# AY-Liu/Image-Editing-Framework

Hardware: AMD Instinct MI355X
Metric: denoising steps/sec (SD1.5 512x512 P2P edit step, UNet batch 4) (higher is better)
Workload: dtype f16x3; 1 GPU; sd15 UNet (859.5M params) P2P AttentionRefine edit step, 2 prompts x CFG = batch 4, 64x64 latents (512x512 px), 50-step DDIM, guidance 7.5, cross 0.8 / self 0.4, per-step null-text unconditional embeddings (P2P_NTI, edit_real.py); one independent edit per GPU; precision mode f16x3: fp32 storage; every contraction on split operands: hi + lo fp16 halves of each fp32 element, Ah Bh + Al Bh + Ah Bl =

## Files before the change

### image-editing-framework_amd/control.py

```python
from typing import Optional

import torch

from . import hip

XL = 96


def _step_hook(c):
    fn = getattr(c, "between_steps", None) or getattr(c, "after_step", None)
    if fn is not None:
        fn()


def advance_controller(c):
    c.cur_att_layer += 1
    uncond = c.num_att_layers if getattr(c, "LOW_RESOURCE", False) else 0
    if c.cur_att_layer == c.num_att_layers + uncond:
        c.cur_att_layer = 0
        c.cur_step += 1
        _step_hook(c)


class StepCounter:
# ... 21 lines not shown
        self.cond_only = bool(cond_only)
        self.batch = num_prompts if cond_only else 2 * num_prompts
        self.num_steps = num_steps
        self.self_window = self_window
        self.self_max_tokens = self_max_tokens
        self.captured = False
        self.muted = False
        dev = self.device
        self.step = torch.zeros(1, dtype=torch.int32, device=dev)
        B, Bp = self.batch, num_prompts
        if kind == "p2p":
            slots = Bp - 1
            assert mt.shape == (slots, XL, XL) and coef_table.shape == (num_steps + 1, slots, 2, XL)
            self.mt = mt.to(device=dev, dtype=torch.float16).contiguous()
            self.mt32 = mt.to(device=dev, dtype=torch.float32).contiguous()
            self.coef_table = coef_table.to(device=dev, dtype=torch.float32).contiguous()
            self.coef_cur = torch.zeros(slots, 2, XL, dtype=torch.float32, device=dev)
            ct = coef_table.detach().float()
            self.coef_bound = float((ct[:, :, 0].abs() + ct[:, :, 1].abs()).max()) if ct.numel() else 1.0
            off = 0 if cond_only else Bp
            es = torch.full((B,), -1, dtype=torch.int32)
            sl = torch.zeros(B, dtype=torch.int32)
            for k in range(slots):
                es[off + 1 + k] = off
                sl[off + 1 + k] = k
            self.edit_src, self.edit_slot = es.to(dev), sl.to(dev)
            ident = torch.arange(B, dtype=torch.int32)
            repl = ident.clone()
            repl[off + 1:] = off
            tab = ident.repeat(num_steps + 1, 1)
# ... 42 lines not shown
                    hip.map_split_scale(self.coef_bound))
        if self.kind == "masactrl":
            return ("masactrl", tuple(sorted(self.masa_layers)), (max(self.masa_steps) + 2) if self.masa_steps else 1)
        if self.kind == "pnp":
            idx = {id(m): m._exec_index for m in unet.attention_modules()}
            inj = (unet.up_blocks[1].resnets[0 if unet.cfg.addition_embed else 1]._inject is self
                   if len(unet.up_blocks) > 1 else False)
            return ("pnp", tuple(sorted(idx[i] for i in self.pnp_layers)), self.num_steps, bool(inj))
        return (self.kind,)

    def load_from(self, other: "ControlPlan", B: int):
        self.controller = other.controller
        if self.kind == "p2p":
            self.mt.copy_(other.mt)
            self.mt32.copy_(other.mt32)
            self.coef_table.copy_(other.coef_table)
            self.coef_bound = other.coef_bound
            self.self_table.copy_(other.self_table)
            self.self_window = other.self_window
        elif self.kind == "masactrl":
            other.prepare(B)
            self.masa_steps = set(other.masa_steps)
            self._masa[B][0].copy_(other._masa[B][0])
        elif self.kind == "pnp":
            other.prepare(B)
            self.pnp_qk_steps, self.pnp_conv_steps = other.pnp_qk_steps, other.pnp_conv_steps
            self._pnp[B][0].copy_(other._pnp[B][0])
            self._pnp[B][2].copy_(other._pnp[B][2])

    def applies(self, B: int) -> bool:
# ... 61 lines not shown
        if self.kind == "p2p" and self.applies(B) and N <= self.self_max_tokens:
            return self.self_cur, self.self_cur, None
        if self.kind == "masactrl" and not self.muted and (attn._exec_index // 2) in self.masa_layers:
            cur = self._masa[B][1]
            return None, cur, cur
        if self.kind == "pnp" and not self.muted and id(attn) in self.pnp_layers:
            cur = self._pnp[B][1]
            return cur, cur, None
        return None, None, None

    def feature_source(self, B: int):
        if self.kind == "pnp" and not self.muted and B in self._pnp:
            return self._pnp[B][3]
        return None

    def cross_edit(self, B: int, attn):
        if self.kind == "p2p" and self.applies(B):
            mt = self.mt32 if attn.to_q.weight.dtype == torch.float32 else self.mt
            args = dict(edit_src=self.edit_src, edit_slot=self.edit_slot, mt=mt, coef=self.coef_cur)
            if attn.to_q.weight.dtype == torch.float32:
                args["coef_bound"] = self.coef_bound
            return args
        return {}
```

### image-editing-framework_amd/denoise.py

```python
import os
from typing import Dict, List, Optional

import torch

from . import hip

REUSE_GRAPHS = os.environ.get("IEF_REUSE_GRAPHS", "1") == "1"
_POOL: Dict[tuple, list] = {}
_POOL_CAP = 8


def _check_finite(lat, unet):
    if not bool(torch.isfinite(lat).all()):
        mode = getattr(unet, "precision", "f16")
        hint = ("an operand left the fp16 range (|x| > 65504): run this model with precision=\"f32\" (IEF_PRECISION=f32 / --precision f32), "
                "the fp32-input MFMA has the fp32 range" if mode != "f32" else "check the inputs / weights")
        raise FloatingPointError(f"non-finite latents after the denoising loop (precision={mode}): {hint}")


class FusedDenoiser:
    def __init__(self, model, context: torch.Tensor, num_latents: int, latent_hw, guidance_scale: Optional[float],
                 mode: str = "denoise", uncond_list: Optional[List[torch.Tensor]] = None, use_graph: bool = True,
                 added_cond_kwargs=None):
        self.model, self.unet, self.sched = model, model.unet, model.scheduler
# ... 55 lines not shown
            if self.ctx is None:
                self.ctx = torch.zeros_like(ctx16)
        else:
            put("ctx", ctx16.clone())

    def _key(self, context, uncond_list):
        plan = self.unet._plan
        return (id(self.unet), self.mode, self.Bp, tuple(self.lat.shape[-2:]), self.cfg, tuple(context.shape),
                None if uncond_list is None else len(uncond_list), len(self.sched.timesteps),
                None if plan is None else plan.signature(self.unet), getattr(self.unet, "attn_key_splits", 1))

    def rebind(self, context, guidance_scale, uncond_list, added_cond_kwargs=None):
        self._fill(context, guidance_scale, uncond_list, added_cond_kwargs)
        if self.ctx_table is None:
            with hip.f32_contraction(getattr(self.unet, "contract", "f32")):
                for m, kv in self._keep:
                    hip.gemm(self.ctx, m.w_kv, out=kv)
        fresh = self.unet._plan
        if self.plan is not None:
            self.plan.load_from(fresh, self.B)
            self.plan.sync_step()
        self.step.zero_()
        self._done = 0

    def _step_body(self):
        hip.select_step(self.temb_table, self.temb_cur, self.step)
        hip.select_step(self.coef_table, self.coef_cur, self.step)
        if self.ctx_table is not None:
            hip.select_step(self.ctx_table, self.ctx, self.step)
        if self.cfg:
            self.lat_in[: self.Bp].copy_(self.lat)
            self.lat_in[self.Bp:].copy_(self.lat)
# ... 35 lines not shown
            self._step_body()
        self.lat.copy_(saved)
        self.step.zero_()
        if plan is not None:
            plan.sync_step()

    def start(self, latents: torch.Tensor):
        self.lat.copy_(latents.to(self.lat.device).float().expand_as(self.lat))
        self.step.zero_()
        self._done = 0
        if self.use_graph and self.graph is None:
            self._capture()
        elif not self.use_graph:
            self._set_kv_cache(self.ctx_table is None)
        if getattr(self, "_keep", None) is None or not self._pooled_started:
            self._keep = [(m, m._kv) for m in self.unet.attention_modules() if m.is_cross and m._kv is not None]
            self._pooled_started = True
        if self.plan is not None and self.graph is not None:
            self.plan.sync_step()

    def rewind(self, latents: Optional[torch.Tensor] = None):
        if latents is not None:
            self.lat.copy_(latents.to(self.lat.device).float().expand_as(self.lat))
        self.step.zero_()
        self._done = 0
        if self.plan is not None:
            self.plan.sync_step()

    def step_once(self):
        if self._done >= self.num_steps:
            raise IndexError(f"step {self._done} is past the {self.num_steps}-step schedule this loop was built for; "
# ... 193 lines not shown
```

### image-editing-framework_amd/hip.py

```python
import ctypes
import os
from ctypes import POINTER, Structure, byref, c_char_p, c_float, c_int, c_longlong, c_void_p

import torch

ABI_VERSION = 4
_LIB_PATH = os.environ.get("IEF_HIP_LIB") or os.path.join(os.path.dirname(os.path.abspath(__file__)), "libief_hip.so")
_lib = None


class HipExtensionMissing(RuntimeError):
    pass


class IefGemmParams(Structure):
    _fields_ = [
        ("A", c_void_p), ("A2", c_void_p), ("W", c_void_p), ("Out", c_void_p),
        ("bias", c_void_p), ("rowvec", c_void_p), ("residual", c_void_p),
        ("M", c_int), ("N", c_int), ("K", c_int),
        ("lda", c_int), ("ldw", c_int), ("ldo", c_int), ("ldr", c_int),
        ("strideA", c_longlong), ("strideW", c_longlong), ("strideO", c_longlong), ("strideR", c_longlong),
        ("H", c_int), ("Wd", c_int), ("C1", c_int), ("C2", c_int), ("Ho", c_int), ("Wo", c_int),
        ("stride", c_int), ("ups", c_int), ("batch_images", c_int),
        ("rows_per_batch", c_int), ("out_scale", c_float), ("tile_hint", c_int),
# ... 107 lines not shown
        ("rstat_slots", c_int), ("rstat_cnt", c_int), ("ln_eps", c_float),
    ]


EXPORTS = [
    "ief_abi_version", "ief_target_arch", "ief_gemm_f16", "ief_conv3x3_f16", "ief_conv_in_f32",
    "ief_conv_out_f32", "ief_gn_splits", "ief_groupnorm_silu_f16", "ief_layernorm_f16", "ief_geglu_f16",
    "ief_attn_flash_f16", "ief_attn_cross_p2p_f16", "ief_attn_probs_f16", "ief_attn_apply_f16",
    "ief_cfg_ddim_step_f32", "ief_timestep_embedding_f16", "ief_silu_f16", "ief_cast_f32_to_f16",
    "ief_cast_f16_to_f32", "ief_select_step", "ief_advance_step", "ief_add_f16", "ief_struct_size",
    "ief_softmax_rows_f16", "ief_transpose_f16", "ief_pointwise_f32",
    "ief_attn_bwd_delta_f32", "ief_attn_bwd_f16", "ief_groupnorm_bwd_f16", "ief_layernorm_bwd_f16", "ief_geglu_il_f16",
    "ief_geglu_il_bwd_f16", "ief_zero_insert2x_f16", "ief_pool2x2_sum_f16", "ief_conv_out_bwd_f32",
    "ief_nti_loss_grad_f32", "ief_nti_adam_f32", "ief_gemm_tile_bn", "ief_gather_rows_f16",
    "ief_attn_map_loss_bwd_f16", "ief_axpy_f32", "ief_map_loss_blocks", "ief_groupnorm_cstat_f16", "ief_gemm_tile_bm",
    "ief_gemm_f32", "ief_softmax_rows_f32", "ief_p2p_cross_edit_f32", "ief_attn_cross_p2p_f32", "ief_groupnorm_silu_f32", "ief_layernorm_f32",
    "ief_add_f32", "ief_silu_f32", "ief_geglu_il_f32", "ief_timestep_embedding_f32", "ief_gather_rows_f32",
    "ief_conv_in_f32act", "ief_conv_out_f32act", "ief_image_u8", "ief_gemm_f32_bn", "ief_attn_flash_f32", "ief_gemm_x3_bn", "ief_gemm_x3_bm", "ief_gemm_x3_bn_k", "ief_gemm_x3_set_variant", "ief_x3_split_weights", "ief_groupnorm_f32_ws_floats", "ief_groupnorm_silu_f32_ws", "ief_groupnorm_bwd_f32_ws_floats", "ief_groupnorm_bwd_f32_ws",
    "ief_groupnorm_bwd_f32", "ief_layernorm_bwd_f32", "ief_geglu_il_bwd_f32", "ief_zero_insert2x_f32", "ief_pool2x2_sum_f32",
    "ief_conv_out_bwd_f32w", "ief_softmax_bwd_rows_f32", "ief_transpose_batched_f32", "ief_map_loss_rows_blocks",
    "ief_map_loss_rows_f32", "ief_nti_adam_f32g",
    "ief_gemm_x3p", "ief_gemm_x3p_tile_bm", "ief_gemm_x3p_tile_bn", "ief_gemm_x3p_tile_wn", "ief_x3_split_act", "ief_groupnorm_silu_x3p_ws", "ief_layernorm_x3p", "ief_groupnorm_silu_x3p_small", "ief_groupnorm_silu_reg", "ief_groupnorm_reg_fits", "ief_attn_bwd_x3", "ief_attn_bwd_delta_f32in",
    "ief_attn_flash_ws_floats",
]


def lib_path() -> str:
    return _LIB_PATH


def load():
# ... 49 lines not shown
                                                                                              c_int, c_void_p]
    lib.ief_layernorm_bwd_f16.argtypes = [c_void_p] * 5 + [c_int, c_int, c_float, c_void_p]
    lib.ief_geglu_il_f16.argtypes = [c_void_p, c_void_p, c_int, c_int, c_void_p]
    lib.ief_geglu_il_bwd_f16.argtypes = [c_void_p, c_void_p, c_void_p, c_int, c_int, c_void_p]
    lib.ief_zero_insert2x_f16.argtypes = [c_void_p, c_void_p] + [c_int] * 4 + [c_void_p]
    lib.ief_pool2x2_sum_f16.argtypes = [c_void_p, c_void_p] + [c_int] * 4 + [c_void_p]
    lib.ief_conv_out_bwd_f32.argtypes = [c_void_p] * 3 + [c_int] * 5 + [c_void_p]
    lib.ief_nti_loss_grad_f32.argtypes = [c_void_p] * 7 + [c_int, c_float, c_void_p]
    lib.ief_nti_adam_f32.argtypes = [c_void_p] * 8 + [c_int, c_void_p]
    lib.ief_gather_rows_f16.argtypes = [c_void_p, c_void_p, c_void_p, c_int, c_longlong, c_void_p]
    lib.ief_gemm_f32.argtypes = [POINTER(IefGemmF32Params), c_void_p]
    lib.ief_softmax_rows_f32.argtypes = [c_void_p, c_longlong, c_int, c_void_p]
    lib.ief_attn_flash_f32.argtypes = [POINTER(IefAttnF32Params), c_void_p]
    lib.ief_p2p_cross_edit_f32.argtypes = [c_void_p] * 5 + [c_int] * 4 + [c_void_p]
    lib.ief_attn_cross_p2p_f32.argtypes = [POINTER(IefAttnF32Params)] + [c_void_p] * 5
    lib.ief_groupnorm_silu_f32.argtypes = [c_void_p, c_void_p, c_int, c_int, c_void_p, c_void_p, c_void_p, c_int, c_int, c_int,
                                           c_float, c_int, c_void_p]
    lib.ief_gemm_x3_bm.argtypes = [c_int, c_int]
    lib.ief_gemm_x3_bn_k.argtypes = [c_int, c_int, c_int]
    if os.environ.get("IEF_X3_WIDE"):
        lib.ief_gemm_x3_set_variant.argtypes = [c_int]
        lib.ief_gemm_x3_set_variant(int(os.environ["IEF_X3_WIDE"]))
    lib.ief_x3_split_weights.argtypes = [c_void_p, c_void_p, c_longlong, c_float, c_void_p]
    lib.ief_groupnorm_bwd_f32.argtypes = [c_void_p, c_void_p, c_int, c_int] + [c_void_p] * 6 + [c_int, c_int, c_int, c_float, c_int, c_void_p]
    lib.ief_layernorm_bwd_f32.argtypes = [c_void_p] * 5 + [c_longlong, c_int, c_float, c_void_p]
    lib.ief_geglu_il_bwd_f32.argtypes = [c_void_p] * 3 + [c_longlong, c_int, c_void_p]
    lib.ief_zero_insert2x_f32.argtypes = [c_void_p, c_void_p, c_int, c_int, c_int, c_int, c_void_p]
    lib.ief_pool2x2_sum_f32.argtypes = [c_void_p, c_void_p, c_int, c_int, c_int, c_int, c_void_p]
    lib.ief_conv_out_bwd_f32w.argtypes = [c_void_p] * 3 + [c_int] * 5 + [c_void_p]
    lib.ief_softmax_bwd_rows_f32.argtypes = [c_void_p, c_void_p, c_longlong, c_int, c_float, c_void_p]
# ... 1811 lines not shown
```

### image-editing-framework_amd/planes.py

```python
import os
from ctypes import byref

import torch

from . import hip
from .hip import IefGemmX3pParams, _check, _dev32, _ptr, _stream, _Timed, _zeros

ACT_SCALE = 1.0
W_SCALE = hip.X3_SCALE_W


class Planes:
    __slots__ = ("t",)

    def __init__(self, t):
        if not (isinstance(t, torch.Tensor) and t.dtype == torch.float16 and t.dim() >= 2 and t.shape[0] == 2 and t.stride(-1) == 1):
            raise TypeError("Planes: expected an fp16 tensor [2, ...] with a contiguous last dimension")
        if not t.is_cuda:
            raise TypeError("Planes: device tensor expected (no CPU path)")
        self.t = t

    @staticmethod
    def empty(*shape, device):
        return Planes(torch.empty(2, *shape, dtype=torch.float16, device=device))
# ... 518 lines not shown
        op, _ = attn_out_args(p, B, N, C, q.device)
    else:
        if out is None:
            out = torch.empty(B, N, C, dtype=torch.float32, device=q.device)
        p.Out, p.sOb, p.ldo = hip._act32(out, "out").data_ptr(), out.stride(0), out.stride(1)
    S = 1 if key_splits == 1 else attn_key_splits(B, heads, N, L, d, setting=key_splits)
    name, nbytes = f"attn_flash_x3p_kernel<{d}>", 4.0 * B * heads * d * (2 * N + 2 * L)
    if S > 1:
        nws = lib.ief_attn_flash_ws_floats(B, heads, N, L, d, S)
        ws = torch.empty(nws, dtype=torch.float32, device=q.device)
        p.key_splits, p.ws, p.ws_floats = S, ws.data_ptr(), nws
        name, nbytes = f"attn_flash_x3p_kernel<{d}, split {S}> + attn_flash_x3p_combine_kernel", nbytes + 8.0 * nws
    with _Timed(name, 4.0 * B * heads * N * L * d, nbytes):
        _check(lib.ief_attn_flash_f32(byref(p), _stream()), "ief_attn_flash_f32 (planes)")
    return op if out_planes else out
```

### image-editing-framework_amd/unet.py

```python
import math
import os
from typing import Dict, Optional

import torch
from torch import nn

from . import hip, planes
from .config import UNetConfig


FOLD_LN = os.environ.get("IEF_FOLD_LN", "1") == "1"
KV_ONE_GEMM = os.environ.get("IEF_KV_ONE_GEMM", "1") == "1"


def _fold_ln(w16, bias32, gamma, beta):
    wf = w16.float()
    wp = (wf * gamma[None, :]).half().contiguous()
    b = wf @ beta
    if bias32 is not None:
        b = b + bias32
    return wp, b.contiguous(), wp.float().sum(1).contiguous()


class UNetOutput(dict):

    def __getattr__(self, k):
        try:
# ... 87 lines not shown
            self.to_q, self.to_k, self.to_v = (Linear(self.w_qkv[i * dim:(i + 1) * dim]) for i in range(3))
            self.w_kv = None
        self.to_out = nn.ModuleList([
            Linear(_f16(sd[f"{prefix}.to_out.0.weight"], dev), _f32(sd[f"{prefix}.to_out.0.bias"], dev)), Dropout()])
        self.spatial_norm = None
        self.group_norm = None
        self.norm_cross = None
        self.residual_connection = False
        self.rescale_output_factor = 1.0
        self.processor = None
        self._plan = None
        self.map_out = None
        self._kv_key, self._kv = None, None
        self.cache_kv = True
        self._kv_view = None
        self.ln_w = self.ln_b = self.ln_c1 = None
        self.ln_eps = 1e-5
        self.attn_key_splits = 1

    def fold_layernorm(self, norm):
        w = self.w_qkv if self.w_qkv is not None else self.to_q.weight
        self.ln_w, self.ln_b, self.ln_c1 = _fold_ln(w, None, norm.weight, norm.bias)
        self.ln_eps = norm.eps

    def prepare_attention_mask(self, attention_mask, target_length, batch_size, out_dim=3):
        if attention_mask is not None:
            raise NotImplementedError("attention masks are not on the reference path (always None)")
        return None

    def head_to_batch_dim(self, t, out_dim=3):
# ... 25 lines not shown

    def is_native(self) -> bool:
        f = self.__dict__.get("forward")
        return (f is None or getattr(f, "__func__", None) is Attention.forward) and self.processor is None

    def context_kv(self, ctx):
        if self._kv_view is not None:
            return self._kv_view
        if not self.cache_kv:
            return hip.gemm(ctx, self.w_kv)
        key = (ctx, ctx._version)
        if self._kv_key is None or self._kv_key[0] is not ctx or self._kv_key[1] != ctx._version:
            self._kv = hip.gemm(ctx, self.w_kv)
            self._kv_key = key
        return self._kv

    def forward(self, hidden_states, encoder_hidden_states=None, attention_mask=None, temb=None, residual=None,
                ln_stats=None, want_stats=False, **cross_attention_kwargs):
        if self.processor is not None:
            return self.processor(self, hidden_states, encoder_hidden_states=encoder_hidden_states,
                                  attention_mask=attention_mask, **cross_attention_kwargs)
        x = hidden_states
        B, N, C = x.shape
        self.last_tokens = N
        plan = self._plan
        ln = None if ln_stats is None else (ln_stats, self.ln_c1, self.ln_eps)
        if encoder_hidden_states is None:
            qkv = hip.gemm(x, self.w_qkv) if ln is None else hip.gemm(x, self.ln_w, bias=self.ln_b, ln=ln)
            q, k, v = qkv[..., :C], qkv[..., C:2 * C], qkv[..., 2 * C:]
            qs = ks = vs = None
# ... 26 lines not shown
        w_in, b_in, ln = (self.w_qkv if ctx is None else self.to_q.weight), None, None
        if ln_stats is not None:
            w_in, b_in, ln = self.ln3.w, self.ln3.bias, (ln_stats, self.ln3.colsum, self.ln3.eps)
        if ctx is None:
            qs = ks = vs = None
            if plan is not None:
                qs, ks, vs = plan.self_sources(B, N, self)
            if planes.FLASH_PLANES and self.dim_head in planes.FLASH_PLANES_DIMS:
                qkv = planes.gemm(xp, w_in, bias=b_in, ln=ln, out=False, out_planes=True)
                o = planes.attn_flash(qkv[..., :C], qkv[..., C:2 * C], qkv[..., 2 * C:], self.heads, self.scale, q_src=qs,
                                      k_src=ks, v_src=vs, key_splits=self.attn_key_splits)
            else:
                qkv = planes.gemm(xp, w_in, bias=b_in, ln=ln)
                o = hip.attn_flash(qkv[..., :C], qkv[..., C:2 * C], qkv[..., 2 * C:], self.heads, self.scale, q_src=qs, k_src=ks,
                                   v_src=vs, out_planes=True)
        else:
            q = planes.gemm(xp, w_in, bias=b_in, ln=ln)
            kv = self.context_kv(ctx)
            args = plan.cross_edit(B, self) if plan is not None else {}
            if self.map_out is not None:
                hip.attn_probs(q, kv[..., :C], self.heads, self.scale, out=self.map_out)
            o = hip.attn_cross_p2p(q, kv[..., :C], kv[..., C:], self.heads, self.scale, out_planes=True, **args)
        if plan is not None:
            plan.layer_done(self)
        lin = self.to_out[0]
        if want_stats:
            return planes.gemm(o, lin.weight, bias=lin.bias, residual=residual, out=True, out_planes=True, row_stats=True)
        return planes.gemm(o, lin.weight, bias=lin.bias, residual=residual)


# ... 478 lines not shown
        x = sample if sample.dtype == torch.float32 else sample.float()
        x = x.contiguous()
        B = x.shape[0]
        ctx = encoder_hidden_states
        if ctx.dtype != self.dtype:
            ctx = self._ctx_f16(ctx)
        if temb_row is None:
            t = torch.as_tensor(timestep).to(device=self._device, dtype=torch.float32).reshape(-1)[:1].contiguous()
            temb_row = self.time_rows(t, self.aug_embedding(added_cond_kwargs))
        trow = lambda r: temb_row[:, r.temb_slot[0]:r.temb_slot[0] + r.temb_slot[1]].contiguous()
        if self._plan is not None:
            self._plan.begin_forward(B)
        cross = self._cross_modules()
        per_step_kv = KV_ONE_GEMM and bool(cross) and not cross[0].cache_kv and all(m.is_native() for m in cross)
        if per_step_kv:
            kv_all = hip.gemm(ctx, self._kv_all_weight())
            off = 0
            for m in cross:
                m._kv_view = kv_all[..., off:off + 2 * m.inner_dim]
                off += 2 * m.inner_dim

        def tap(name, v):
            if taps is not None:
                taps[name] = v.float().permute(0, 3, 1, 2).cpu()

        if self.x3p:
            eps = self._trunk_x3p(x, trow, ctx, tap)
            if per_step_kv:
                for m in cross:
                    m._kv_view = None
            if self._plan is not None:
                self._plan.end_forward(B)
            return (eps,) if not return_dict else UNetOutput(sample=eps)
        h, hs = hip.conv_in(x, self.conv_in.weight, self.conv_in.bias), None
        tap("conv_in", h)
        skips = [(h, hs)]
        for bi, blk in enumerate(self.down_blocks):
            for j, res in enumerate(blk.resnets):
                h, hs = res(h, trow(res), cstat=hs, col_stats=True)
                if blk.has_cross_attention:
                    h, hs = blk.attentions[j](h, ctx, cstat=hs, col_stats=True)
                skips.append((h, hs))
            if blk.downsamplers is not None:
                h, hs = blk.downsamplers[0](h, col_stats=True)
                skips.append((h, hs))
# ... 3 lines not shown
        h, hs = self.mid_block.resnets[1](h, trow(self.mid_block.resnets[1]), cstat=hs, col_stats=True)
        tap("mid", h)
        for bi, blk in enumerate(self.up_blocks):
            for j, res in enumerate(blk.resnets):
                sk, sks = skips.pop()
                h, hs = res(h, trow(res), skip=sk, cstat=hs, cstat_skip=sks, col_stats=True)
                if blk.has_cross_attention:
                    h, hs = blk.attentions[j](h, ctx, cstat=hs, col_stats=True)
            if blk.upsamplers is not None:
                h, hs = blk.upsamplers[0](h, col_stats=True)
            tap(f"up{bi}", h)
        h = self.conv_norm_out(h, silu=True, cstat=hs)
        eps = hip.conv_out(h, self.conv_out.weight, self.conv_out.bias)
        if per_step_kv:
            for m in cross:
                m._kv_view = None
        if self._plan is not None:
            self._plan.end_forward(B)
        if not return_dict:
            return (eps,)
        return UNetOutput(sample=eps)

    def _trunk_x3p(self, x, trow, ctx, tap):
        h = hip.conv_in(x, self.conv_in.weight, self.conv_in.bias)
        hp = planes.split(h)
        tap("conv_in", h)
        skips = [(h, hp)]
        for bi, blk in enumerate(self.down_blocks):
            for j, res in enumerate(blk.resnets):
                attn = blk.has_cross_attention
                h, hp = res.forward_x3p(h, hp, trow(res), want_planes=not attn)
# ... 62 lines not shown
```

### include/ief_hip.h

```cpp
#ifndef IEF_HIP_H
#define IEF_HIP_H
#include <stdint.h>

#ifdef __HIPCC__
typedef _Float16 ief_half;
#else
typedef uint16_t ief_half;
#endif

#ifdef __cplusplus
extern "C" {
#endif

#define IEF_ABI_VERSION 4
int ief_abi_version(void);
const char* ief_target_arch(void);
int ief_struct_size(int which);

typedef struct IefGemmParams {
    const ief_half* A;
    const ief_half* A2;
    const ief_half* W;
    ief_half* Out;
    const float* bias;
// ... 130 lines not shown
    int ldp;
    float p_scale;
    const ief_half* Qp; const ief_half* Kp; const ief_half* Vp;
    long long planeQ, planeK, planeV;
    const void* zeros;
    float* lse;
    int key_splits; float* ws; long long ws_floats;
} IefAttnF32Params;
int ief_attn_flash_f32(const IefAttnF32Params* p, void* stream);
long long ief_attn_flash_ws_floats(int B, int heads, int N, int L, int d, int key_splits);
int ief_softmax_rows_f32(float* x, long long rows, int L, void* stream);
int ief_p2p_cross_edit_f32(float* P, const int* edit_src, const int* edit_slot, const float* MT, const float* coef, int B,
                           int heads, int N, int L, void* stream);
int ief_attn_cross_p2p_f32(const IefAttnF32Params* p, const int* edit_src, const int* edit_slot, const float* MT, const float* coef,
                           void* stream);
int ief_groupnorm_silu_f32(const float* x, const float* x2, int C1, int C2, float* out, const float* gamma, const float* beta,
                           int B, int HW, int groups, float eps, int silu, void* stream);
long long ief_groupnorm_f32_ws_floats(int B, int HW, int C);
int ief_groupnorm_silu_f32_ws(const float* x, const float* x2, int C1, int C2, float* out, const float* gamma, const float* beta,
                              int B, int HW, int groups, float eps, int silu, float* ws, long long ws_floats, void* stream);
int ief_groupnorm_reg_fits(int C1, int C2, int HW, int groups);
int ief_groupnorm_silu_reg(const float* x, const float* x2, int C1, int C2, float* out, ief_half* outp, long long plane,
                           const float* gamma, const float* beta, int B, int HW, int groups, float eps, int silu, void* stream);
long long ief_groupnorm_bwd_f32_ws_floats(int B, int HW, int C);
int ief_groupnorm_bwd_f32_ws(const float* x, const float* x2, int C1, int C2, const float* dy, const float* add, float* dx, float* dx2,
                             const float* gamma, const float* beta, int B, int HW, int groups, float eps, int silu, float* ws,
                             long long ws_floats, void* stream);
int ief_layernorm_f32(const float* x, float* out, const float* gamma, const float* beta, long long rows, int C, float eps,
                      void* stream);
int ief_groupnorm_silu_x3p_ws(const float* x, const float* x2, int C1, int C2, float* out, ief_half* outp, long long plane,
// ... 134 lines not shown
```

Baseline: 73.81 steps/s.

## Add fused split-plane cross-attention kernel with P2P edit for x3p path

Adds a HIP kernel that runs cross-attention with the P2P mapper edit directly on pre-split hi/lo fp16 planes of Q, K, V and the mapper table. The QK, mapper and PV contractions all use three-product MFMA chains, and the output is written as planes. The context K/V projection is also produced in planes once per step, so cross-attention no longer splits fp32 operands or runs separate edit and softmax passes. In exchange it adds a large kernel with LDS staging and extra split bookkeeping, and accuracy depends on the chosen plane scaling.

```diff
diff --git a/image-editing-framework_amd/control.py b/image-editing-framework_amd/control.py
--- a/image-editing-framework_amd/control.py
+++ b/image-editing-framework_amd/control.py
@@ -2,7 +2,7 @@
 
 import torch
 
-from . import hip
+from . import hip, planes
 
 XL = 96
 
@@ -59,6 +59,7 @@
             assert mt.shape == (slots, XL, XL) and coef_table.shape == (num_steps + 1, slots, 2, XL)
             self.mt = mt.to(device=dev, dtype=torch.float16).contiguous()
             self.mt32 = mt.to(device=dev, dtype=torch.float32).contiguous()
+            self.mtp = planes.table_planes(self.mt32)
             self.coef_table = coef_table.to(device=dev, dtype=torch.float32).contiguous()
             self.coef_cur = torch.zeros(slots, 2, XL, dtype=torch.float32, device=dev)
             ct = coef_table.detach().float()
@@ -131,6 +132,7 @@
         if self.kind == "p2p":
             self.mt.copy_(other.mt)
             self.mt32.copy_(other.mt32)
+            self.mtp.copy_(other.mtp)
             self.coef_table.copy_(other.coef_table)
             self.coef_bound = other.coef_bound
             self.self_table.copy_(other.self_table)
@@ -222,8 +224,11 @@
             return self._pnp[B][3]
         return None
 
-    def cross_edit(self, B: int, attn):
+    def cross_edit(self, B: int, attn, as_planes: bool = False):
         if self.kind == "p2p" and self.applies(B):
+            if as_planes:
+                return dict(edit_src=self.edit_src, edit_slot=self.edit_slot, mtp=self.mtp, coef=self.coef_cur,
+                            coef_bound=self.coef_bound)
             mt = self.mt32 if attn.to_q.weight.dtype == torch.float32 else self.mt
             args = dict(edit_src=self.edit_src, edit_slot=self.edit_slot, mt=mt, coef=self.coef_cur)
             if attn.to_q.weight.dtype == torch.float32:
diff --git a/image-editing-framework_amd/csrc/cross_p2p_x3p.hip b/image-editing-framework_amd/csrc/cross_p2p_x3p.hip
--- /dev/null
+++ b/image-editing-framework_amd/csrc/cross_p2p_x3p.hip
@@ -0,0 +1,296 @@
+#include "ief_common.h"
+#include "ief_params.h"
+#include "x3_common.h"
+
+template <int D>
+__device__ __forceinline__ int xc_swz(int row) { return D == 64 ? (row & 7) : D == 160 ? ((row >> 2) & 3) : 0; }
+
+template <int D, int NWV>
+__global__ __launch_bounds__(64 * NWV) void attn_cross_p2p_x3p_kernel(const IefAttnF32Params p, const int* __restrict__ edit_src,
+                                                                       const int* __restrict__ edit_slot,
+                                                                       const half_t* __restrict__ MTP,
+                                                                       const float* __restrict__ coef) {
+    constexpr int DG = (D + 15) / 16;
+    constexpr int DT = (D + 31) / 32;
+    constexpr int CPR = D / 8;
+    constexpr int KPL = ((96 * D * 2 + 1023) / 1024) * 512;
+    constexpr int NPC = KPL / 512;
+    constexpr int MPL = 96 * 96;
+    constexpr bool SHARE = D > 80;
+    constexpr float SP = 16384.f, SM = 256.f;
+    __shared__ __attribute__((aligned(1024))) half_t smem_x[(SHARE ? 2 : 3) * 2 * KPL + 2 * MPL];
+    __shared__ float cf[2 * 96];
+    half_t* const Ks = smem_x;
+    half_t* const Kt = smem_x + 2 * KPL;
+    half_t* const Vt = SHARE ? Ks : smem_x + 4 * KPL;
+    half_t* const Mt = smem_x + (SHARE ? 4 : 6) * KPL;
+    const float SPE = p.p_scale > 0.f ? p.p_scale : SP;
+    const int tid = threadIdx.x, lane = tid & 63;
+    const int wid = __builtin_amdgcn_readfirstlane(tid >> 6);
+    const int li = lane & 31, lh = lane >> 5;
+    const int nqb = gridDim.x;
+    const int lid = xcd_remap(blockIdx.x + nqb * blockIdx.y, nqb * gridDim.y);
+    const int bh = lid / nqb, qb = lid - bh * nqb, b = bh / p.heads, h = bh - b * p.heads;
+    const int src = edit_src ? edit_src[b] : -1;
+    const bool edited = src >= 0;
+    const int qi = qb * (32 * NWV) + wid * 32 + li;
+    const int nt = (p.L + 31) / 32;
+    const float sc2 = p.scale * 1.44269504088896341f;
+    const char* zp = (const char*)p.zeros;
+
+    const int npc = (nt * 32 * CPR + 63) / 64;
+    auto stage = [&](const half_t* gb, long long plane, int ld, half_t* lds) {
+        for (int q = wid; q < 2 * NPC; q += NWV) {
+            const int pl = q >= NPC ? 1 : 0, j = q - pl * NPC;
+            if (j < npc) {
+                const int c = 64 * j + lane;
+                const int row = c / CPR, ch = (c - row * CPR) ^ xc_swz<D>(row);
+                const char* g = row < p.L ? (const char*)(gb + pl * plane + (long long)row * ld) + ch * 16 : zp;
+                x3_glds16(g, lds + pl * KPL + j * 512);
+            }
+        }
+    };
+    auto kbase = [&](int br) { return p.Kp + (long long)br * p.sKb + (long long)h * D; };
+    stage(kbase(edited ? src : b), p.planeK, p.ldk, edited ? Ks : Kt);
+    if (edited) {
+        stage(kbase(b), p.planeK, p.ldk, Kt);
+        const half_t* mt = MTP + (long long)edit_slot[b] * (2 * MPL);
+        for (int q = wid; q < 36; q += NWV) {
+            const int pl = q >= 18 ? 1 : 0, j = q - pl * 18;
+            const int c = 64 * j + lane;
+            const int row = c / 12, ch = (c - row * 12) ^ ((row >> 2) & 3);
+            x3_glds16((const char*)(mt + pl * MPL + row * 96) + ch * 16, Mt + pl * MPL + j * 512);
+        }
+        for (int i = tid; i < 192; i += 64 * NWV) cf[i] = coef[(long long)edit_slot[b] * 192 + i];
+    }
+    const half_t* Vg = p.Vp + (long long)b * p.sVb + (long long)h * D;
+    if (!(SHARE && edited)) stage(Vg, p.planeV, p.ldv, Vt);
+
+    auto load_q = [&](int br, half8_t (&qh)[DG], half8_t (&ql)[DG]) {
+        const half_t* Q = p.Qp + (long long)br * p.sQb + (long long)h * D;
+#pragma unroll
+        for (int g = 0; g < DG; ++g) {
+            const int d0 = g * 16 + 8 * lh;
+            if (qi < p.N && d0 < D) {
+                qh[g] = *(const half8_t*)(Q + (long long)qi * p.ldq + d0);
+                ql[g] = *(const half8_t*)(Q + p.planeQ + (long long)qi * p.ldq + d0);
+            } else {
+#pragma unroll
+                for (int j = 0; j < 8; ++j) { qh[g][j] = 0; ql[g][j] = 0; }
+            }
+        }
+    };
+    int koff[DG];
+#pragma unroll
+    for (int g = 0; g < DG; ++g) {
+        const int chunk = (g * 16 + 8 * lh < D) ? 2 * g + lh : 0;
+        koff[g] = li * D + ((chunk ^ xc_swz<D>(li)) << 3);
+    }
+    auto probs = [&](const half8_t (&qh)[DG], const half8_t (&ql)[DG], const half_t* Kh, f32x16 (&P)[3]) {
+        const half_t* Kl = Kh + KPL;
+        float mx = -INFINITY;
+#pragma unroll
+        for (int t = 0; t < 3; ++t) {
+#pragma unroll
+            for (int r = 0; r < 16; ++r) P[t][r] = -INFINITY;
+            if (t < nt) {
+                f32x16 sacc;
+#pragma unroll
+                for (int r = 0; r < 16; ++r) sacc[r] = 0.f;
+#pragma unroll
+                for (int g = 0; g < DG; ++g) {
+                    const half8_t kh = *(const half8_t*)(Kh + t * 32 * D + koff[g]);
+                    const half8_t kl = *(const half8_t*)(Kl + t * 32 * D + koff[g]);
+                    sacc = __builtin_amdgcn_mfma_f32_32x32x16_f16(kl, qh[g], sacc, 0, 0, 0);
+                    sacc = __builtin_amdgcn_mfma_f32_32x32x16_f16(kh, ql[g], sacc, 0, 0, 0);
+                    sacc = __builtin_amdgcn_mfma_f32_32x32x16_f16(kh, qh[g], sacc, 0, 0, 0);
+                }
+                if ((t + 1) * 32 > p.L) {
+#pragma unroll
+                    for (int r = 0; r < 16; ++r) {
+                        const int key = t * 32 + (r & 3) + 8 * (r >> 2) + 4 * lh;
+                        P[t][r] = key < p.L ? sacc[r] * sc2 : -INFINITY;
+                        mx = fmaxf(mx, P[t][r]);
+                    }
+                } else {
+#pragma unroll
+                    for (int r = 0; r < 16; ++r) { P[t][r] = sacc[r] * sc2; mx = fmaxf(mx, P[t][r]); }
+                }
+            }
+        }
+        mx = fmaxf(mx, __shfl_xor(mx, 32));
+        float ls = 0.f;
+#pragma unroll
+        for (int t = 0; t < 3; ++t)
+#pragma unroll
+            for (int r = 0; r < 16; ++r) { P[t][r] = __builtin_amdgcn_exp2f(P[t][r] - mx); ls += P[t][r]; }
+        ls += __shfl_xor(ls, 32);
+        const float inv = 1.0f / ls;
+#pragma unroll
+        for (int t = 0; t < 3; ++t)
+#pragma unroll
+            for (int r = 0; r < 16; ++r) P[t][r] *= inv;
+    };
+    auto split_p = [&](const f32x16& P, int s, half8_t& ph, half8_t& pl, float sp) {
+#pragma unroll
+        for (int c2 = 0; c2 < 2; ++c2) {
+            const f32x4 v = {P[8 * s + 4 * c2], P[8 * s + 4 * c2 + 1], P[8 * s + 4 * c2 + 2], P[8 * s + 4 * c2 + 3]};
+            half4 hh, ll;
+            split4(v, sp, hh, ll);
+#pragma unroll
+            for (int j = 0; j < 4; ++j) { ph[4 * c2 + j] = hh[j]; pl[4 * c2 + j] = ll[j]; }
+        }
+    };
+
+    half8_t qh[DG], ql[DG];
+    load_q(edited ? src : b, qh, ql);
+    asm volatile("s_waitcnt vmcnt(0)" ::: "memory");
+    __syncthreads();
+    f32x16 T[3];
+    if (edited) {
+        f32x16 Ps[3];
+        probs(qh, ql, Ks, Ps);
+        load_q(b, qh, ql);
+        if (SHARE) {
+            __syncthreads();
+            stage(Vg, p.planeV, p.ldv, Vt);
+        }
+        half8_t ph[6], pl[6];
+#pragma unroll
+        for (int s = 0; s < 6; ++s) split_p(Ps[s >> 1], s & 1, ph[s], pl[s], SP);
+        const half_t* Mh = Mt;
+        const half_t* Ml = Mt + MPL;
+        const int msw = (li >> 2) & 3;
+#pragma unroll
+        for (int wt = 0; wt < 3; ++wt) {
+#pragma unroll
+            for (int r = 0; r < 16; ++r) T[wt][r] = 0.f;
+#pragma unroll
+            for (int s = 0; s < 6; ++s) {
+                const int o0 = (wt * 32 + li) * 96 + (((2 * s) ^ msw) << 3) + 4 * lh;
+                const int o1 = (wt * 32 + li) * 96 + (((2 * s + 1) ^ msw) << 3) + 4 * lh;
+                half8_t mh, ml;
+                const half4 a0 = *(const half4*)(Mh + o0), a1 = *(const half4*)(Mh + o1);
+                const half4 b0 = *(const half4*)(Ml + o0), b1 = *(const half4*)(Ml + o1);
+#pragma unroll
+                for (int j = 0; j < 4; ++j) { mh[j] = a0[j]; mh[4 + j] = a1[j]; ml[j] = b0[j]; ml[4 + j] = b1[j]; }
+                T[wt] = __builtin_amdgcn_mfma_f32_32x32x16_f16(ml, ph[s], T[wt], 0, 0, 0);
+                T[wt] = __builtin_amdgcn_mfma_f32_32x32x16_f16(mh, pl[s], T[wt], 0, 0, 0);
+                T[wt] = __builtin_amdgcn_mfma_f32_32x32x16_f16(mh, ph[s], T[wt], 0, 0, 0);
+            }
+        }
+    }
+    f32x16 P[3];
+    probs(qh, ql, Kt, P);
+    if (edited) {
+        const float invt = 1.0f / (SM * SP);
+#pragma unroll
+        for (int t = 0; t < 3; ++t)
+#pragma unroll
+            for (int r = 0; r < 16; ++r) {
+                const int w = t * 32 + (r & 3) + 8 * (r >> 2) + 4 * lh;
+                P[t][r] = cf[w] * (T[t][r] * invt) + cf[96 + w] * P[t][r];
+            }
+        if (SHARE) {
+            asm volatile("s_waitcnt vmcnt(0)" ::: "memory");
+            __syncthreads();
+        }
+    }
+    const half_t* Vh = Vt;
+    const half_t* Vl = Vt + KPL;
+    const int L16 = lane & 15;
+    const int vrow = 4 * lh + (L16 >> 2);
+    int voff[DT];
+#pragma unroll
+    for (int tt = 0; tt < DT; ++tt) {
+        int col = 32 * tt + 16 * ((lane >> 4) & 1) + 4 * (L16 & 3);
+        if (col >= D) col = 0;
+        voff[tt] = col;
+    }
+    f32x16 o[DT];
+#pragma unroll
+    for (int tt = 0; tt < DT; ++tt)
+#pragma unroll
+        for (int r = 0; r < 16; ++r) o[tt][r] = 0.f;
+#pragma unroll
+    for (int t = 0; t < 3; ++t) {
+        if (t < nt) {
+#pragma unroll
+            for (int s = 0; s < 2; ++s) {
+                half8_t ph, pl;
+                split_p(P[t], s, ph, pl, SPE);
+                const int r0 = t * 32 + 16 * s + vrow;
+#pragma unroll
+                for (int tt = 0; tt < DT; ++tt) {
+                    const int c = voff[tt];
+                    const int o0 = r0 * D + ((((c >> 3) ^ xc_swz<D>(r0)) << 3) | (c & 7));
+                    const int o1 = (r0 + 8) * D + ((((c >> 3) ^ xc_swz<D>(r0 + 8)) << 3) | (c & 7));
+                    const half4 a0 = x3_lds_tr_read(Vh + o0), a1 = x3_lds_tr_read(Vh + o1);
+                    const half4 b0 = x3_lds_tr_read(Vl + o0), b1 = x3_lds_tr_read(Vl + o1);
+                    half8_t vh, vl;
+#pragma unroll
+                    for (int j = 0; j < 4; ++j) { vh[j] = a0[j]; vh[4 + j] = a1[j]; vl[j] = b0[j]; vl[4 + j] = b1[j]; }
+                    o[tt] = __builtin_amdgcn_mfma_f32_32x32x16_f16(vl, ph, o[tt], 0, 0, 0);
+                    o[tt] = __builtin_amdgcn_mfma_f32_32x32x16_f16(vh, pl, o[tt], 0, 0, 0);
+                    o[tt] = __builtin_amdgcn_mfma_f32_32x32x16_f16(vh, ph, o[tt], 0, 0, 0);
+                }
+            }
+        }
+    }
+    const float inv = 1.0f / SPE;
+    float* O = p.Out ? p.Out + (long long)b * p.sOb + (long long)h * D : nullptr;
+    half_t* OP = p.OutP ? p.OutP + (long long)b * p.sOPb + (long long)h * D : nullptr;
+    if (qi < p.N) {
+#pragma unroll
+        for (int tt = 0; tt < DT; ++tt)
+#pragma unroll
+            for (int g = 0; g < 4; ++g) {
+                const int d = tt * 32 + 8 * g + 4 * lh;
+                if (d < D) {
+                    const f32x4 v = {o[tt][4 * g] * inv, o[tt][4 * g + 1] * inv, o[tt][4 * g + 2] * inv, o[tt][4 * g + 3] * inv};
+                    if (O) *(f32x4*)(O + (long long)qi * p.ldo + d) = v;
+                    if (OP) {
+                        half4 hh, ll;
+                        split4(v, 1.0f, hh, ll);
+                        half_t* op = OP + (long long)qi * p.ldp + d;
+                        *(half4*)op = hh;
+                        *(half4*)(op + p.planeO) = ll;
+                    }
+                }
+            }
+    }
+}
+
+extern "C" int ief_attn_cross_p2p_x3p(const IefAttnF32Params* pp, const int* edit_src, const int* edit_slot, const ief_half* MTP,
+                                      const float* coef, int waves, void* stream) {
+    if (!pp) return IEF_EINVAL;
+    const IefAttnF32Params& p = *pp;
+    if (!p.Qp || !p.Kp || !p.Vp || !p.zeros || (!p.Out && !p.OutP) || p.q_src || p.k_src || p.v_src) return IEF_EINVAL;
+    if (p.p_scale != 0.f && !(p.p_scale >= 1.f && p.p_scale <= 16384.f)) return IEF_EINVAL;
+    if (edit_src && (!edit_slot || !MTP || !coef)) return IEF_EINVAL;
+    if (p.B <= 0 || p.heads <= 0 || p.N <= 0 || p.L <= 0 || p.L > 96) return IEF_ESHAPE;
+    if (waves == 0) waves = 4;
+    if (waves != 1 && waves != 2 && waves != 4 && waves != 8) return IEF_EINVAL;
+    if ((p.ldq & 7) || (p.ldk & 7) || (p.ldv & 7) || (p.sQb & 7) || (p.sKb & 7) || (p.sVb & 7) || (p.planeQ & 7) || (p.planeK & 7) ||
+        (p.planeV & 7) || (((uintptr_t)p.Qp | (uintptr_t)p.Kp | (uintptr_t)p.Vp | (uintptr_t)p.zeros | (uintptr_t)(MTP ? MTP : p.zeros)) & 15))
+        return IEF_EALIGN;
+    if (p.Out && ((p.ldo & 3) || (p.sOb & 3) || ((uintptr_t)p.Out & 15))) return IEF_EALIGN;
+    if (p.OutP && ((p.ldp & 3) || (p.sOPb & 3) || (p.planeO & 3) || ((uintptr_t)p.OutP & 7))) return IEF_EALIGN;
+    hipStream_t st = (hipStream_t)stream;
+    const long long nqb = ((long long)p.N + 32 * waves - 1) / (32 * waves), nbh = (long long)p.B * p.heads;
+    if (nbh > 65535 || nqb > 0x7fffffffLL) return IEF_ESHAPE;
+    const dim3 grid((unsigned)nqb, (unsigned)nbh);
+    const half_t* mtp = (const half_t*)MTP;
+#define CROSSP_GO(D_, W_) hipLaunchKernelGGL((attn_cross_p2p_x3p_kernel<D_, W_>), grid, dim3(64 * W_), 0, st, p, edit_src, edit_slot, mtp, coef)
+#define CROSSP_D(D_) do { switch (waves) { case 1: CROSSP_GO(D_, 1); break; case 2: CROSSP_GO(D_, 2); break; \
+                                           case 4: CROSSP_GO(D_, 4); break; default: CROSSP_GO(D_, 8); break; } } while (0)
+    switch (p.d) {
+        case 40: CROSSP_D(40); break;
+        case 64: CROSSP_D(64); break;
+        case 80: CROSSP_D(80); break;
+        case 160: CROSSP_D(160); break;
+        default: return IEF_ESHAPE;
+    }
+    IEF_LAUNCH_CHECK();
+    return IEF_OK;
+}
diff --git a/image-editing-framework_amd/denoise.py b/image-editing-framework_amd/denoise.py
--- a/image-editing-framework_amd/denoise.py
+++ b/image-editing-framework_amd/denoise.py
@@ -3,7 +3,7 @@
 
 import torch
 
-from . import hip
+from . import hip, planes
 
 REUSE_GRAPHS = os.environ.get("IEF_REUSE_GRAPHS", "1") == "1"
 _POOL: Dict[tuple, list] = {}
@@ -93,8 +93,12 @@
         self._fill(context, guidance_scale, uncond_list, added_cond_kwargs)
         if self.ctx_table is None:
             with hip.f32_contraction(getattr(self.unet, "contract", "f32")):
-                for m, kv in self._keep:
+                for m, kv, kvp in self._keep:
                     hip.gemm(self.ctx, m.w_kv, out=kv)
+                    if kvp is not None:
+                        planes.split(kv, out=kvp)
+                        if m._kvp is kvp and m._kvp_of is kv:
+                            m._kvp_ver = kv._version
         fresh = self.unet._plan
         if self.plan is not None:
             self.plan.load_from(fresh, self.B)
@@ -160,7 +164,8 @@
         elif not self.use_graph:
             self._set_kv_cache(self.ctx_table is None)
         if getattr(self, "_keep", None) is None or not self._pooled_started:
-            self._keep = [(m, m._kv) for m in self.unet.attention_modules() if m.is_cross and m._kv is not None]
+            self._keep = [(m, m._kv, m._kvp if m._kvp_of is m._kv else None) for m in self.unet.attention_modules()
+                          if m.is_cross and m._kv is not None]
             self._pooled_started = True
         if self.plan is not None and self.graph is not None:
             self.plan.sync_step()
diff --git a/image-editing-framework_amd/hip.py b/image-editing-framework_amd/hip.py
--- a/image-editing-framework_amd/hip.py
+++ b/image-editing-framework_amd/hip.py
@@ -145,7 +145,7 @@
     "ief_geglu_il_bwd_f16", "ief_zero_insert2x_f16", "ief_pool2x2_sum_f16", "ief_conv_out_bwd_f32",
     "ief_nti_loss_grad_f32", "ief_nti_adam_f32", "ief_gemm_tile_bn", "ief_gather_rows_f16",
     "ief_attn_map_loss_bwd_f16", "ief_axpy_f32", "ief_map_loss_blocks", "ief_groupnorm_cstat_f16", "ief_gemm_tile_bm",
-    "ief_gemm_f32", "ief_softmax_rows_f32", "ief_p2p_cross_edit_f32", "ief_attn_cross_p2p_f32", "ief_groupnorm_silu_f32", "ief_layernorm_f32",
+    "ief_gemm_f32", "ief_softmax_rows_f32", "ief_p2p_cross_edit_f32", "ief_attn_cross_p2p_f32", "ief_attn_cross_p2p_x3p", "ief_groupnorm_silu_f32", "ief_layernorm_f32",
     "ief_add_f32", "ief_silu_f32", "ief_geglu_il_f32", "ief_timestep_embedding_f32", "ief_gather_rows_f32",
     "ief_conv_in_f32act", "ief_conv_out_f32act", "ief_image_u8", "ief_gemm_f32_bn", "ief_attn_flash_f32", "ief_gemm_x3_bn", "ief_gemm_x3_bm", "ief_gemm_x3_bn_k", "ief_gemm_x3_set_variant", "ief_x3_split_weights", "ief_groupnorm_f32_ws_floats", "ief_groupnorm_silu_f32_ws", "ief_groupnorm_bwd_f32_ws_floats", "ief_groupnorm_bwd_f32_ws",
     "ief_groupnorm_bwd_f32", "ief_layernorm_bwd_f32", "ief_geglu_il_bwd_f32", "ief_zero_insert2x_f32", "ief_pool2x2_sum_f32",
@@ -225,6 +225,7 @@
     lib.ief_attn_flash_f32.argtypes = [POINTER(IefAttnF32Params), c_void_p]
     lib.ief_p2p_cross_edit_f32.argtypes = [c_void_p] * 5 + [c_int] * 4 + [c_void_p]
     lib.ief_attn_cross_p2p_f32.argtypes = [POINTER(IefAttnF32Params)] + [c_void_p] * 5
+    lib.ief_attn_cross_p2p_x3p.argtypes = [POINTER(IefAttnF32Params)] + [c_void_p] * 4 + [c_int, c_void_p]
     lib.ief_groupnorm_silu_f32.argtypes = [c_void_p, c_void_p, c_int, c_int, c_void_p, c_void_p, c_void_p, c_int, c_int, c_int,
                                            c_float, c_int, c_void_p]
     lib.ief_gemm_x3_bm.argtypes = [c_int, c_int]
diff --git a/image-editing-framework_amd/planes.py b/image-editing-framework_amd/planes.py
--- a/image-editing-framework_amd/planes.py
+++ b/image-editing-framework_amd/planes.py
@@ -556,3 +556,73 @@
     with _Timed(name, 4.0 * B * heads * N * L * d, nbytes):
         _check(lib.ief_attn_flash_f32(byref(p), _stream()), "ief_attn_flash_f32 (planes)")
     return op if out_planes else out
+
+
+CROSS_PLANES = os.environ.get("IEF_X3P_CROSS", "0") == "1"
+CROSS_PLANES_DIMS = (40, 64, 80, 160)
+CROSS_WAVES = (1, 2, 4, 8)
+
+
+def cross_waves(B, heads, N, d, cus=None) -> int:
+    if cus is None:
+        cus = torch.cuda.get_device_properties(torch.cuda.current_device()).multi_processor_count
+    for w in (8, 4, 2):
+        if -(-N // (32 * w)) * B * heads >= cus:
+            return w
+    return 1
+
+
+def table_planes(mt32):
+    x = mt32.to(torch.float32) * W_SCALE
+    hi = x.to(torch.float16)
+    lo = (x - hi.to(torch.float32)).to(torch.float16)
+    return torch.stack([hi, lo], 1).contiguous()
+
+
+def attn_cross_p2p(q, k, v, heads, scale, edit_src=None, edit_slot=None, mtp=None, coef=None, out=None, out_planes=True,
+                   coef_bound=1.0, waves=None):
+    lib = hip.load()
+    for t, nm in ((q, "q"), (k, "k"), (v, "v")):
+        if not isinstance(t, Planes) or t.dim() != 3:
+            raise TypeError(f"planes.attn_cross_p2p: {nm} must be Planes [B, rows, heads*d]")
+    B, N, C = q.shape
+    L, d = k.shape[1], C // heads
+    if d not in CROSS_PLANES_DIMS or L > 96:
+        raise ValueError(f"planes.attn_cross_p2p: head dim {d} / {L} keys have no planes instantiation")
+    p = hip.IefAttnF32Params()
+    for t, nm in ((q, "Q"), (k, "K"), (v, "V")):
+        h_ = t.hi
+        if h_.stride(2) != 1 or (h_.shape[0] > 1 and h_.stride(0) != h_.shape[1] * h_.stride(1)):
+            raise ValueError("planes.attn_cross_p2p: operands must be [B, rows, heads*d] with batch stride rows * ld")
+        setattr(p, nm + "p", h_.data_ptr())
+        setattr(p, "plane" + nm, t.plane)
+    p.ldq, p.ldk, p.ldv = q.hi.stride(1), k.hi.stride(1), v.hi.stride(1)
+    p.sQb, p.sKb, p.sVb = q.hi.stride(0), k.hi.stride(0), v.hi.stride(0)
+    p.B, p.heads, p.N, p.L, p.d, p.scale = B, heads, N, L, d, scale
+    p.x3, p.zeros = 1, _zeros(q.device)
+    es = sl = None
+    if edit_src is not None:
+        if (not isinstance(mtp, torch.Tensor) or mtp.dtype != torch.float16 or mtp.dim() != 4 or tuple(mtp.shape[1:]) != (2, 96, 96)
+                or not mtp.is_contiguous() or not mtp.is_cuda):
+            raise ValueError("planes.attn_cross_p2p: mtp must be the contiguous fp16 planes [slots,2,96,96] of the table (table_planes)")
+        if _dev32(coef, "coef").shape[-1] != 96 or not coef.is_contiguous():
+            raise ValueError("planes.attn_cross_p2p: coef must be contiguous fp32 [slots,2,96]")
+        es, sl = hip._devi32(edit_src, "edit_src"), hip._devi32(edit_slot, "edit_slot")
+        p.p_scale = hip.map_split_scale(coef_bound)
+    op = None
+    if out_planes:
+        op, _ = attn_out_args(p, B, N, C, q.device)
+    else:
+        if out is None:
+            out = torch.empty(B, N, C, dtype=torch.float32, device=q.device)
+        if hip._act32(out, "out").stride(2) != 1 or (B > 1 and out.stride(0) != out.shape[1] * out.stride(1)) or tuple(out.shape[::2]) != (B, C) or out.shape[1] < N:
+            raise ValueError("planes.attn_cross_p2p: out must be fp32 [B, >= N, heads*d] with batch stride rows * ld")
+        p.Out, p.sOb, p.ldo = out.data_ptr(), out.stride(0), out.stride(1)
+    w = cross_waves(B, heads, N, d) if waves is None else int(waves)
+    if w not in CROSS_WAVES:
+        raise ValueError(f"planes.attn_cross_p2p: waves must be one of {CROSS_WAVES}")
+    nedit = 2.0 * B * heads * N * 96 * 96 if edit_src is not None else 0.0
+    with _Timed(f"attn_cross_p2p_x3p_kernel<{d}, {w}>", 4.0 * B * heads * N * L * d + nedit, 4.0 * B * heads * d * (2 * N + 2 * L)):
+        _check(lib.ief_attn_cross_p2p_x3p(byref(p), _ptr(es), _ptr(sl), _ptr(mtp) if es is not None else None,
+                                          _ptr(coef) if es is not None else None, w, _stream()), "ief_attn_cross_p2p_x3p")
+    return op if out_planes else out
diff --git a/image-editing-framework_amd/unet.py b/image-editing-framework_amd/unet.py
--- a/image-editing-framework_amd/unet.py
+++ b/image-editing-framework_amd/unet.py
@@ -11,6 +11,7 @@
 
 FOLD_LN = os.environ.get("IEF_FOLD_LN", "1") == "1"
 KV_ONE_GEMM = os.environ.get("IEF_KV_ONE_GEMM", "1") == "1"
+KV_PLANES = os.environ.get("IEF_X3P_KV_PLANES", "1") == "1"
 
 
 def _fold_ln(w16, bias32, gamma, beta):
@@ -128,6 +129,8 @@
         self._kv_key, self._kv = None, None
         self.cache_kv = True
         self._kv_view = None
+        self._kvp_view = None
+        self._kvp, self._kvp_of, self._kvp_ver = None, None, -1
         self.ln_w = self.ln_b = self.ln_c1 = None
         self.ln_eps = 1e-5
         self.attn_key_splits = 1
@@ -183,6 +186,16 @@
             self._kv = hip.gemm(ctx, self.w_kv)
             self._kv_key = key
         return self._kv
+
+    def context_kv_planes(self, ctx):
+        if self._kvp_view is not None:
+            return self._kvp_view
+        kv = self.context_kv(ctx)
+        if not self.cache_kv or self._kv_view is not None:
+            return planes.split(kv)
+        if self._kvp is None or self._kvp_of is not kv or self._kvp_ver != kv._version:
+            self._kvp, self._kvp_of, self._kvp_ver = planes.split(kv), kv, kv._version
+        return self._kvp
 
     def forward(self, hidden_states, encoder_hidden_states=None, attention_mask=None, temb=None, residual=None,
                 ln_stats=None, want_stats=False, **cross_attention_kwargs):
@@ -239,6 +252,12 @@
                 qkv = planes.gemm(xp, w_in, bias=b_in, ln=ln)
                 o = hip.attn_flash(qkv[..., :C], qkv[..., C:2 * C], qkv[..., 2 * C:], self.heads, self.scale, q_src=qs, k_src=ks,
                                    v_src=vs, out_planes=True)
+        elif (planes.CROSS_PLANES and self.map_out is None and self.dim_head in planes.CROSS_PLANES_DIMS and ctx.shape[1] <= 96
+              and hip.X3_FUSE_CROSS):
+            qp = planes.gemm(xp, w_in, bias=b_in, ln=ln, out=False, out_planes=True)
+            kvp = self.context_kv_planes(ctx)
+            args = plan.cross_edit(B, self, as_planes=True) if plan is not None else {}
+            o = planes.attn_cross_p2p(qp, kvp[..., :C], kvp[..., C:], self.heads, self.scale, **args)
         else:
             q = planes.gemm(xp, w_in, bias=b_in, ln=ln)
             kv = self.context_kv(ctx)
@@ -747,10 +766,19 @@
         cross = self._cross_modules()
         per_step_kv = KV_ONE_GEMM and bool(cross) and not cross[0].cache_kv and all(m.is_native() for m in cross)
         if per_step_kv:
-            kv_all = hip.gemm(ctx, self._kv_all_weight())
+            kv_planes = (self.x3p and planes.CROSS_PLANES and KV_PLANES and hip.X3_FUSE_CROSS and ctx.shape[1] <= 96
+                         and all(m.map_out is None and m.dim_head in planes.CROSS_PLANES_DIMS for m in cross)
+                         and planes.supported(self._kv_all_weight().shape[0], ctx.shape[-1]))
+            if kv_planes:
+                kv_all = planes.gemm(planes.split(ctx), self._kv_all_weight(), out=False, out_planes=True)
+            else:
+                kv_all = hip.gemm(ctx, self._kv_all_weight())
             off = 0
             for m in cross:
-                m._kv_view = kv_all[..., off:off + 2 * m.inner_dim]
+                if kv_planes:
+                    m._kvp_view = kv_all[..., off:off + 2 * m.inner_dim]
+                else:
+                    m._kv_view = kv_all[..., off:off + 2 * m.inner_dim]
                 off += 2 * m.inner_dim
 
         def tap(name, v):
@@ -761,7 +789,7 @@
             eps = self._trunk_x3p(x, trow, ctx, tap)
             if per_step_kv:
                 for m in cross:
-                    m._kv_view = None
+                    m._kv_view = m._kvp_view = None
             if self._plan is not None:
                 self._plan.end_forward(B)
             return (eps,) if not return_dict else UNetOutput(sample=eps)
@@ -795,7 +823,7 @@
         eps = hip.conv_out(h, self.conv_out.weight, self.conv_out.bias)
         if per_step_kv:
             for m in cross:
-                m._kv_view = None
+                m._kv_view = m._kvp_view = None
         if self._plan is not None:
             self._plan.end_forward(B)
         if not return_dict:
diff --git a/include/ief_hip.h b/include/ief_hip.h
--- a/include/ief_hip.h
+++ b/include/ief_hip.h
@@ -168,6 +168,8 @@
                            int heads, int N, int L, void* stream);
 int ief_attn_cross_p2p_f32(const IefAttnF32Params* p, const int* edit_src, const int* edit_slot, const float* MT, const float* coef,
                            void* stream);
+int ief_attn_cross_p2p_x3p(const IefAttnF32Params* p, const int* edit_src, const int* edit_slot, const ief_half* MTP,
+                           const float* coef, int waves, void* stream);
 int ief_groupnorm_silu_f32(const float* x, const float* x2, int C1, int C2, float* out, const float* gamma, const float* beta,
                            int B, int HW, int groups, float eps, int silu, void* stream);
 long long ief_groupnorm_f32_ws_floats(int B, int HW, int C);
```

After: 73.78 steps/s. About the same (-0.0%).
